# SamShue/EKF_SLAM

Measured on AMD Instinct MI355X. Metric: EKF update-steps/sec at N landmarks; HBM GB/s on (I−KH)P vs roofline, higher is better.
Workload: dtype f64

## Files before the change

### ekf_slam_amd/csrc/abi.hip

```cpp
#include "../../include/ekfslam.h"

#include <hip/hip_runtime.h>

#include <dlfcn.h>

#include <cstdio>
#include <cstdlib>
#include <algorithm>
#include <cmath>
#include <cstring>
#include <new>
#include <string>
#include <vector>

#include "device_math.h"
#include "flush32_pipe.h"
#include "kernels.h"
#include "layout.h"

struct KernelTimer {
    bool enabled = false;
    std::vector<hipEvent_t> ev;
    size_t used = 0;
};
// ... 38 lines not shown
    int32_t storage = 0;
    int32_t cur = 0;
    int32_t batch = 1;
    int32_t npend = 0;
    int32_t pstart = 0;
    bool async_flush = false;
    void *tilebuf[2] = { nullptr, nullptr };
    int32_t base = 0;
    int32_t nfrozen = 0;
    bool inflight = false;
    hipStream_t flush_stream = nullptr;
    hipEvent_t ev_pairs = nullptr, ev_flushed = nullptr, ev_rows = nullptr;
    hipEvent_t ev_xchg = nullptr;
    bool have_pp = false;
    PredictArgs pp;
    std::vector<double> s_host;
    mutable std::vector<std::pair<double, int64_t>> s_sorted, s_tail;
    mutable bool s_sorted_ok = false;
    static constexpr size_t kSortedTail = 2048;
    hipEvent_t throttle_ev[2] = { nullptr, nullptr };
    bool throttle_set[2] = { false, false };
    int throttle_k = 0, since_mark = 0;
    DevState st;
    hipStream_t own_stream = nullptr, stream = nullptr;
    int2 *d_work = nullptr;
    int64_t nwork = 0, work_rows = -1, work_cap = 0;
    char *wl_stage = nullptr;
    size_t wl_stage_bytes = 0;
    hipEvent_t ev_wl = nullptr;
    bool wl_busy = false;
// ... 234 lines not shown
    const bool alternate = force >= 0 ? force != 0 : store > kCacheBytes;
    h->st.tm.reverse = alternate ? (h->st.tm.reverse ^ 1) : 0;
}

int64_t slab_for(const ekf_handle *h, int64_t mm_rows) {
    const int64_t nt = ekf_tiles_for(mm_rows, h->T);
    const int64_t cmax = (nt + h->cfg.world - 1) / h->cfg.world;
    return cmax * h->T * 2;
}

double *corr_send(const ekf_handle *h, int64_t slab) {
    return (h->comm && h->send == h->own_send && h->recv == h->own_recv) ? h->recv + (size_t)h->cfg.rank * (size_t)slab : h->send;
}

int32_t exchange_rccl(ekf_handle *h);
int32_t flush_pending(ekf_handle *h, bool batch_done = false) {
    int32_t rc = retire_inflight(h);
    if (rc) return rc;
    if (h->npend == 0) return EKF_OK;
    rc = refresh_work(h);
    if (rc) return rc;
    next_pass_direction(h);
    bool extracted = false;
    const int64_t hint = h->hint_idx;
    bool pn = false, pn_side = false;
    if (batch_done && !h->pn_idx.empty()) {
        if (h->sharded && !h->pending && h->pn_N == h->N && (h->comm || h->xhook)) {
            const int32_t m = (int32_t)h->pn_idx.size();
            const int64_t slab = slab_for(h, n_mm(h));
            {
                TimedLaunch tl(h, EKF_KERNEL_ROWPANEL);
                HIPCHK(h, launch_rowpanel_next(h->st, h->pn_idx.data(), m, n_mm(h), h->pstart, h->npend, h->send, slab, h->storage, h->stream));
// ... 44 lines not shown
                                  h->storage, h->grid_cap, h->stream, h->dd_kernel, nx.j >= 0 ? &nx : nullptr, &extracted, h->cfg.pass_arith,
                                  h->d_segs ? &h->aux : nullptr));
        h->dd_pairs = h->npend;
    }
    h->npend = 0;
    h->pstart = 0;
    h->pf_valid = pn;
    if (pn_side) HIPCHK(h, hipStreamWaitEvent(h->stream, h->ev_pn_done, 0));
    h->nx_valid = extracted && !pn;
    if (extracted) { h->nx_idx = hint; h->nx_N = h->N; }
    return EKF_OK;
}

int32_t batch_complete(ekf_handle *h) {
    if (!h->async_flush) return flush_pending(h,  true);
    HIPCHK(h, hipEventRecord(h->ev_pairs, h->stream));
    int32_t rc = retire_inflight(h);
    if (rc) return rc;
    rc = refresh_work(h);
    if (rc) return rc;
    HIPCHK(h, hipStreamWaitEvent(h->flush_stream, h->ev_pairs, 0));
    {
        KernelTimer *t = &h->timers[EKF_KERNEL_DOWNDATE];
        hipEvent_t stop = nullptr;
        if (t->enabled) {
            if (t->used + 2 > t->ev.size()) {
                hipEvent_t a, b;
                HIPCHK(h, hipEventCreate(&a)); HIPCHK(h, hipEventCreate(&b));
                t->ev.push_back(a); t->ev.push_back(b);
            }
// ... 48 lines not shown
            continue;
        }
        const bool same = sp.is_new ? v.index == -1 : (int64_t)v.index == sp.idx;
        if (!same) {
            char buf[200];
            snprintf(buf, sizeof buf, "measure: the device association decided %s %d where the host mirror of the signatures "
                     "predicted %s %lld; the state is no longer the reference's", v.index == -1 ? "new landmark" : v.index == -2 ?
                     "(stale winner entries)" : "landmark", (int)v.index, sp.is_new ? "new landmark" : "landmark", (long long)sp.idx);
            rc = fail(h, EKF_ERR_STATE, buf);
        }
    }
    h->lspec.erase(h->lspec.begin(), h->lspec.begin() + (ptrdiff_t)done);
    return rc;
}

int32_t materialize_predict(ekf_handle *h) {
    if (!h->have_pp) return EKF_OK;
    h->have_pp = false;
    PredictArgs a = h->pp;
    a.n_mm = n_mm(h); a.cur = h->cur;
    {
        TimedLaunch tl(h, EKF_KERNEL_PREDICT);
        HIPCHK(h, launch_predict(h->st, a, h->storage, h->stream));
    }
    h->cur ^= 1;
    return EKF_OK;
}

int32_t do_predict(ekf_handle *h, const double u[2]) {
    int32_t rc = materialize_predict(h);
    if (rc) return rc;
// ... 1 lines not shown
    h->have_pp = true;
    static const bool lazy = ekf_tune_int("EKF_LAZY_PREDICT", 1) != 0;
    return lazy ? EKF_OK : materialize_predict(h);
}

int32_t enter(ekf_handle *h) {
    HIPCHK(h, hipSetDevice(h->cfg.device));
    const int32_t rc = verify_loop(h,  true);
    if (rc) return rc;
    return materialize_predict(h);
}

int32_t do_append(ekf_handle *h, const double u[2], const double R[4], const double pos[2], double signature,
                  const DevLoopArgs *dl = nullptr) {
    REQUIRE(h, h->N < h->cap, EKF_ERR_CAPACITY, "append: capacity_landmarks exhausted");
    if (h->inflight) h->appended_inflight = true;
    AppendArgs a;
    a.u0 = u[0]; a.u1 = u[1];
    colmajor2(R, a.R00, a.R01, a.R10, a.R11);
    a.pos0 = pos[0]; a.pos1 = pos[1]; a.signature = signature; a.N = h->N; a.cur = h->cur;
    {
        PredictArgs pa = h->pp;
        pa.n_mm = n_mm(h); pa.cur = h->cur;
        const PredictArgs *fuse = h->have_pp ? &pa : nullptr;
        TimedLaunch tl(h, EKF_KERNEL_APPEND);
        HIPCHK(h, launch_append(h->st, a, h->storage, h->stream, dl, fuse));
        if (fuse) { h->have_pp = false; h->cur ^= 1; }
    }
    if ((int64_t)h->s_host.size() > h->N) { h->s_host.resize((size_t)h->N); h->s_sorted_ok = false; }
    h->s_host.push_back(signature);
    if (h->s_sorted_ok && signature == signature)
        h->s_tail.emplace_back(signature, h->N);
    h->N += 1;
    h->pf_valid = false;
    h->nx_valid = false;
    h->pn_idx.clear();
// ... 134 lines not shown
        }
        int32_t rc = correct_begin(h, z, R, idx);
        if (rc) return rc;
        rc = exchange_rccl(h);
        if (rc) { h->pending = false; return rc; }
        return correct_finish(h);
    }
    REQUIRE(h, idx >= 0 && idx < h->N, EKF_ERR_INDEX, "correct: landmark index outside the state");
    int32_t rc = refresh_work(h);
    if (rc) return rc;
    CorrectArgs a;
    fill_correct_args(h, a, z, R, idx);
    static const bool fuse_small = ekf_tune_int("EKF_FUSE_SMALL", 1) != 0;
    const bool fused = fuse_small && h->batch == 1 && !h->async_flush && h->npend == 0 && a.n_mm <= gather_fuse_max_rows() &&
                       ekf_tiles_for(a.n_mm, h->T) * h->T <= 256;
    {
        TimedLaunch tl(h, EKF_KERNEL_GATHER);
        const PredictArgs *fuse = h->have_pp ? &h->pp : nullptr;
        HIPCHK(h, launch_gather(h->st, a, fuse, h->storage, h->stream, fused));
        h->have_pp = false;
    }
    if (fused) {
        h->cur ^= 1;
        h->st.dcur ^= 1;
        snprintf(h->dd_kernel, sizeof h->dd_kernel, "k_gather<%s,fused downdate>", h->storage == EKF_STORE_F64 ? "double" : "float");
        h->dd_pairs = 1;
        return throttle_step(h);
    }
    return finish_step(h);
}

int32_t do_correct_dev(ekf_handle *h, const double z[2], const double R[4], int64_t idx, const DevLoopArgs &dl) {
    REQUIRE(h, idx >= 0 && idx < h->N, EKF_ERR_INDEX, "correct: landmark index outside the state");
    int32_t rc = refresh_work(h);
    if (rc) return rc;
    CorrectArgs a;
    fill_correct_args(h, a, z, R, idx);
    if (h->sharded) {
        REQUIRE(h, !h->pending, EKF_ERR_STATE, "correct: an exchange is pending");
        h->slab = slab_for(h, a.n_mm);
        {
            TimedLaunch tl(h, EKF_KERNEL_ROWPANEL);
            HIPCHK(h, launch_rowpanel_dev(h->st, a.j, a.n_mm, h->pstart, h->npend, corr_send(h, h->slab), h->storage, h->stream, dl));
        }
        h->nx_valid = false;
        h->pending = true; h->pending_kind = 1; h->x_count = h->slab;
        rc = exchange_rccl(h);
        h->pending = false; h->pending_kind = 0;
        if (rc) return rc;
// ... 51 lines not shown
    return EKF_OK;
}

int32_t collect_decision(ekf_handle *h, AssocHostPartial *set, int32_t nblk, int32_t seq, int64_t N, bool may_poll, int32_t *is_new,
                         int64_t *idx) {
    if (!(may_poll && h->assoc_poll && wait_parts(set, nblk, seq))) {
        HIPCHK(h, hipStreamSynchronize(h->stream));
        __atomic_thread_fence(__ATOMIC_ACQUIRE);
    }
    return reduce_parts(h, set, nblk, seq, N, is_new, idx);
}

int32_t launch_assoc(ekf_handle *h, const double z[3], const double R[4], AssocHostPartial *host_set_dev, int32_t seq,
                     bool exchange = false, bool want_costs = false, bool fold_predict = false) {
    REQUIRE(h, h->N >= 1, EKF_ERR_STATE, "associate: the state holds no landmark (Correspondence.m:29)");
    if (!fold_predict) {
        const int32_t rcp = materialize_predict(h);
        if (rcp) return rcp;
    }
    AssocArgs a;
    a.z0 = z[0]; a.z1 = z[1]; a.z2 = z[2];
    colmajor2(R, a.R00, a.R01, a.R10, a.R11);
    a.s_cost = h->cfg.s_cost; a.s_thresh = h->cfg.s_thresh; a.w_pos = h->cfg.w_pos;
    a.N = h->N; a.cur = h->cur; a.npend = h->npend; a.pstart = h->pstart;
    a.own_only = exchange ? 1 : 0;
    TimedLaunch tl(h, EKF_KERNEL_ASSOCIATE);
    HIPCHK(h, launch_associate(h->st, a, exchange ? (want_costs ? h->send + 4 : nullptr) : h->d_pos_cost, h->d_sig_cost,
                               h->d_partial, h->d_ticket, h->d_decision, exchange ? nullptr : host_set_dev, seq,
                               exchange ? h->send : nullptr, h->storage, h->stream, (fold_predict && h->have_pp) ? &h->pp : nullptr));
    if (fold_predict && h->have_pp) { h->have_pp = false; h->cur ^= 1; }
// ... 1109 lines not shown
```

### ekf_slam_amd/csrc/append.h

```cpp
#pragma once

template <typename TS, bool kPredict = false>
__global__ __launch_bounds__(kBlock) void k_append(DevState st, AppendArgs a, DevLoopArgs dl, PredictArgs pa) {
    __shared__ PredictSmall aps;
    const int cur = a.cur;
    const int out = kPredict ? (cur ^ 1) : cur;
    if constexpr (kPredict) {
        if (threadIdx.x == 0) {
            const double pose[3] = { st.x[cur][0], st.x[cur][1], st.x[cur][2] };
            double prr_in[9];
            for (int i = 0; i < 9; ++i) prr_in[i] = st.prr[cur][i];
            predict_small(pose, prr_in, pa.u0, pa.u1, pa.C, aps);
        }
        __syncthreads();
    }
    if (dl.parts_in != nullptr && blockIdx.x == 0 && threadIdx.x < 64) {
        double dll;
        int dix;
        reduce_partials_wave(dl.parts_in, dl.nblk_in, dl.seq_in, (int)threadIdx.x, dll, dix);
        if (threadIdx.x == 0) store_partial(dl.rec, dll, dix, dl.seq_rec);
    }
    double *__restrict__ x = st.x[out];
    double *__restrict__ s = st.strip[out];
    const double *__restrict__ prr = kPredict ? aps.prr : st.prr[cur];
    TS *__restrict__ tiles = (TS *)st.tiles;
    const int64_t n_mm = 2 * a.N;
    const int64_t c = (int64_t)blockIdx.x * kBlock + threadIdx.x;
    const double th = kPredict ? aps.pose[2] : x[2];
    const double jxr[2][3] = { { 1, 0, -a.u0 * ekfm::sind(th) }, { 0, 1, a.u0 * ekfm::cosd(th) } };
    if (c < n_mm) {
        const double *__restrict__ sin_ = st.strip[cur];
        double s0 = sin_[c], s1 = sin_[st.ldm + c];
        const double s2 = sin_[2 * st.ldm + c];
        if constexpr (kPredict) {
            predict_strip(s0, s1, s2, aps.fa, aps.fb);
            s[c] = s0; s[st.ldm + c] = s1; s[2 * st.ldm + c] = s2;
            x[3 + c] = st.x[cur][3 + c];
        }
        for (int i = 0; i < 2; ++i) {
            const double v = jxr[i][0] * s0 + jxr[i][1] * s1 + jxr[i][2] * s2;
            if (st.tm.mine((n_mm + i) >> st.tm.shift, c >> st.tm.shift))
                pmm_low_store<TS>(tiles, st.tm, n_mm + i, c, v);
        }
    }
    if (c == 0) {
        if constexpr (kPredict) {
            for (int i = 0; i < 9; ++i) { st.prr[out][i] = aps.prr[i]; st.small[12 + i] = aps.Q[i]; }
            for (int i = 0; i < 3; ++i) x[i] = aps.pose[i];
        }
        x[3 + n_mm] = a.pos0;
        x[3 + n_mm + 1] = a.pos1;
        st.s[a.N] = a.signature;
        const double jz[2][2] = { { ekfm::cosd(a.u1), -a.u0 * ekfm::sind(a.u1) },
                                  { ekfm::sind(a.u1),  a.u0 * ekfm::cosd(a.u1) } };
        const double R[2][2] = { { a.R00, a.R01 }, { a.R10, a.R11 } };
        double t[2][3], c1[2][2], t2[2][2], c2[2][2];
        for (int i = 0; i < 2; ++i) for (int j = 0; j < 3; ++j) {
            double acc = 0; for (int k = 0; k < 3; ++k) acc += jxr[i][k] * prr[3 * k + j]; t[i][j] = acc; }
        for (int i = 0; i < 2; ++i) for (int j = 0; j < 2; ++j) {
            double acc = 0; for (int k = 0; k < 3; ++k) acc += t[i][k] * jxr[j][k]; c1[i][j] = acc; }
        for (int i = 0; i < 2; ++i) for (int j = 0; j < 2; ++j) {
            double acc = 0; for (int k = 0; k < 2; ++k) acc += jz[i][k] * R[k][j]; t2[i][j] = acc; }
        for (int i = 0; i < 2; ++i) for (int j = 0; j < 2; ++j) {
            double acc = 0; for (int k = 0; k < 2; ++k) acc += t2[i][k] * jz[j][k]; c2[i][j] = acc; }
        {
            double *__restrict__ dg = st.diag[st.dcur] + 3 * a.N;
            dg[0] = c1[0][0] + c2[0][0]; dg[1] = c1[1][0] + c2[1][0]; dg[2] = c1[1][1] + c2[1][1];
        }
        if (st.tm.mine(n_mm >> st.tm.shift, n_mm >> st.tm.shift)) {
            pmm_low_store<TS>(tiles, st.tm, n_mm, n_mm, c1[0][0] + c2[0][0]);
            pmm_low_store<TS>(tiles, st.tm, n_mm + 1, n_mm, c1[1][0] + c2[1][0]);
            pmm_low_store<TS>(tiles, st.tm, n_mm + 1, n_mm + 1, c1[1][1] + c2[1][1]);
        }
        for (int i = 0; i < 3; ++i) for (int j = 0; j < 2; ++j) {
            double acc = 0; for (int k = 0; k < 3; ++k) acc += prr[3 * i + k] * jxr[j][k];
            s[i * st.ldm + n_mm + j] = acc; }
    }
}
```

### ekf_slam_amd/csrc/gather.h

```cpp
#pragma once

constexpr int kGatherCols = 256;
constexpr int kGatherBlock = kGatherCols + 3 * 64;

__device__ __forceinline__ double lane_bcast(double v, int src) {
    const int lo = __builtin_amdgcn_readlane(__double2loint(v), src), hi = __builtin_amdgcn_readlane(__double2hiint(v), src);
    return __hiloint2double(hi, lo);
}
__device__ __forceinline__ double lane_gather(double v, int src) {
    const int lo = __builtin_amdgcn_ds_bpermute(src << 2, __double2loint(v)), hi = __builtin_amdgcn_ds_bpermute(src << 2, __double2hiint(v));
    return __hiloint2double(hi, lo);
}
__device__ __forceinline__ double lane_xor1(double v) {
    const int lo = __builtin_amdgcn_mov_dpp(__double2loint(v), 0xB1, 0xF, 0xF, true), hi = __builtin_amdgcn_mov_dpp(__double2hiint(v), 0xB1, 0xF, 0xF, true);
    return __hiloint2double(hi, lo);
}
__device__ __forceinline__ void wave_lds_sync() { asm volatile("s_waitcnt lgkmcnt(0)" ::: "memory"); }

constexpr int kFuseMaxRows = 48;
constexpr int kFuseElems = kFuseMaxRows * kFuseMaxRows / 256;

template <typename TS, bool kSharded, bool kPredict, bool kFused = false, bool kDev = false>
__global__ __launch_bounds__(kGatherBlock) void k_gather(DevState st, CorrectArgs a, PanelView pv, PredictArgs pa,
                                                         typename DevLoopParam<kDev>::type dl) {
    static_assert(!kDev || !kFused, "the device loop never drives the small-map fused form");
    __shared__ double pss[24];
    __shared__ SmallSolve sol;
    __shared__ PredictSmall ps;
    __shared__ double pose_sh[3];
    __shared__ int diag_ready;
    __shared__ int staged_cnt;
    __shared__ double2 upatch[kMaxPending * 4];
    const int tid = threadIdx.x;
    const int role = __builtin_amdgcn_readfirstlane(tid >> 6);
    const int lane = tid & 63;
    const int cur = a.cur;
    const double *__restrict__ x = cur ? st.x[1] : st.x[0];
    const double *__restrict__ strip = cur ? st.strip[1] : st.strip[0];
    const double *__restrict__ prr_cur = cur ? st.prr[1] : st.prr[0];
    double *__restrict__ x_nxt = cur ? st.x[0] : st.x[1];
    double *__restrict__ strip_nxt = cur ? st.strip[0] : st.strip[1];
    double *__restrict__ prr_nxt = cur ? st.prr[0] : st.prr[1];
    const TS *__restrict__ tiles = (const TS *)st.tiles;
    int64_t j = a.j;
    const int64_t ldm = st.ldm;
    const int npend = a.npend, pstart = a.pstart;
    if constexpr (kDev) {
        double dll;
        int dix;
        reduce_partials_wave(dl.parts_in, dl.nblk_in, dl.seq_in, lane, dll, dix);
        dix = __builtin_amdgcn_readfirstlane(dix);
        if (dix >= 0 && 2 * (int64_t)dix < a.n_mm) j = 2 * (int64_t)dix;
        if constexpr (kSharded) pv.Ij = j >> st.tm.shift;
        if (blockIdx.x == 0 && tid == kGatherCols + 128) store_partial(dl.rec, dll, dix, dl.seq_rec);
    }

    {
        const double *t_tiles = (const double *)st.tiles;
        asm volatile("" :: "s"(st.ldm), "s"(st.pair_stride), "s"(st.pcap), "s"(st.Gp), "s"(st.Kp), "s"(t_tiles), "s"(st.small),
                     "s"(st.tm.T), "s"(st.tm.shift), "s"(st.tm.world), "s"(st.tm.rank), "s"(a.j), "s"(a.n_mm), "s"(a.npend),
                     "s"(a.pstart));
// ... 4 lines not shown
#define EKF_STAMP() do { stamp[nst++] = clock64(); } while (0)
    EKF_STAMP();
#else
#define EKF_STAMP() do { } while (0)
#endif

    if (role >= 4) {
        double small_v = 0.0;
        if (role == 4) {
            const double *sp = prr_cur;
            if (lane < 9) sp = prr_cur + lane;
            else if (lane < 15) { const int t = (lane - 9) >> 1, b = (lane - 9) & 1; sp = strip + t * ldm + j + b; }
            else if (lane >= 19 && lane < 22) sp = x + (lane - 19);
            else if (lane >= 22 && lane < 24) sp = x + 3 + j + (lane - 22);
            small_v = *sp;
            if (lane == 24) { diag_ready = 0; staged_cnt = 0; }
        } else if (role == 5) {
            const int t = (lane >> 1) & 1, b = lane & 1;
            small_v = st.diag[st.dcur][3 * (j >> 1) + (t > b ? t : b) + (t > b ? b : t)];
        } else {
            small_v = x[lane < 3 ? lane : 3 + j + ((lane - 3) & 1)];
        }
        __builtin_amdgcn_sched_barrier(0);
        asm volatile("s_barrier" ::: "memory");
        EKF_STAMP();
        if (role == 4 && (lane < 15 || (lane >= 19 && lane < 24))) pss[lane] = small_v;
        if (role == 5 && lane < 4) pss[15 + lane] = small_v;
        EKF_STAMP();
        if (role == 5) {
            wave_lds_sync();
            if (lane == 0) *(volatile int *)&diag_ready = 1;
            EKF_STAMP();
        } else if (role == 6) {
            const double bx = lane_bcast(small_v, 0), by = lane_bcast(small_v, 1), bth = lane_bcast(small_v, 2),
                         blx = lane_bcast(small_v, 3), bly = lane_bcast(small_v, 4);
            if (lane == 0) {
                double pose[3] = { bx, by, bth };
                if (kPredict) {
                    const double2 sc2 = sincosd_ni(pose[2] + pa.u1);
                    const double sn2 = sc2.x, cs2 = sc2.y;
                    const double p0 = predict_pose_entry(pose, 0, pa.u0, pa.u1, sn2, cs2), p1 = predict_pose_entry(pose, 1, pa.u0, pa.u1, sn2, cs2),
                                 p2 = predict_pose_entry(pose, 2, pa.u0, pa.u1, sn2, cs2);
                    pose[0] = p0; pose[1] = p1; pose[2] = p2;
                }
                const double d0 = blx - pose[0], d1 = bly - pose[1];
                const double bearing = bearing_ni(d1, d0, pose[2]);
                const double sq = sqrt(d0 * d0 + d1 * d1);
                sol.nu[0] = a.z0 - sq;
                sol.nu[1] = a.z1 - bearing;
            }
        } else {
            double p[24];
#pragma unroll
            for (int i = 0; i < 24; ++i) p[i] = (i >= 15 && i < 19) ? 0.0 : lane_bcast(small_v, i);
// ... 17 lines not shown
                const double wj = EKF_SEL(ej == 0) ? W[0] : (EKF_SEL(ej == 1) ? W[1] : W[2]);
                double e_prr, e_q;
                predict_prr_entry(ei, ej, cj, c2, fa, fb, wi, wj, pa.C, e_prr, e_q);
                double s0 = v0, s1 = v1;
                predict_strip(s0, s1, v2, fa, fb);
                const double e_strip = EKF_SEL(st_t == 0) ? s0 : (EKF_SEL(st_t == 1) ? s1 : v2);
                const double p0 = predict_pose_entry(pose, 0, pa.u0, pa.u1, sn2, cs2), p1 = predict_pose_entry(pose, 1, pa.u0, pa.u1, sn2, cs2),
                             p2 = predict_pose_entry(pose, 2, pa.u0, pa.u1, sn2, cs2);
                pose[0] = p0; pose[1] = p1; pose[2] = p2;
                EKF_STAMP();
                if (lane < 15) pss[lane] = EKF_SEL(is_prr) ? e_prr : e_strip;
                if (lane < 9) ps.Q[lane] = e_q;
                if (lane == 0) { ps.fa = fa; ps.fb = fb; }
            }
            if (lane < 3) pose_sh[lane] = lane == 0 ? pose[0] : lane == 1 ? pose[1] : pose[2];
            SmallSolve so;
            double sq;
            solve_hs(p[22] - pose[0], p[23] - pose[1], sq, so.Hs);
            EKF_STAMP();
            while (*(volatile int *)&diag_ready == 0) { }
            wave_lds_sync();
            const int ra = lane >= 5 ? 1 : 0;
            double hsel[5];
#pragma unroll
            for (int t = 0; t < 5; ++t) hsel[t] = ra ? so.Hs[1][t] : so.Hs[0][t];
            const double e_gs = solve_gs_entry(pss, hsel, lane < 10 ? lane - 5 * ra : 0);
            double GS[2][5];
#pragma unroll
            for (int i = 0; i < 10; ++i) GS[i / 5][i % 5] = lane_bcast(e_gs, i);
            double e_phi;
            {
                const int aa = (lane >> 1) & 1, bb = lane & 1;
                double gsel[5], hb[5];
#pragma unroll
                for (int t = 0; t < 5; ++t) { gsel[t] = aa ? GS[1][t] : GS[0][t]; hb[t] = bb ? so.Hs[1][t] : so.Hs[0][t]; }
                const double Rab = aa == 0 ? (bb == 0 ? a.R00 : a.R01) : (bb == 0 ? a.R10 : a.R11);
// ... 67 lines not shown
        else if (rowpart) {
            const int64_t m = st.tm.T - 1;
            const TS *__restrict__ tp = tiles + st.tm.tile_offset(j >> st.tm.shift, c >> st.tm.shift) + ((j & m) << st.tm.shift) + (c & m);
            m0 = (double)tp[0]; m1 = (double)tp[st.tm.T];
        }
        else if (colpart) pmm_low_pair<TS>(tiles, st.tm, c, j, m0, m1);
        else pmm_low_pair<TS>(tiles, st.tm, j + 1, j, m0, m1);
        s0 = strip[c]; s1 = strip[ldm + c]; s2 = strip[2 * ldm + c];
        xc = x[3 + c];
    }
    double dgc = 0.0, dgl = 0.0;
    if (live) {
        const double *__restrict__ dg = st.diag[st.dcur] + 3 * (c >> 1);
        if (c & 1) { dgl = dg[1]; dgc = dg[2]; } else dgc = dg[0];
    }
    __builtin_amdgcn_sched_barrier(0);
    EKF_STAMP();
    upatch[tid] = up0; upatch[tid + kGatherCols] = up1;
    wave_lds_sync();
    if ((tid & 63) == 0) atomicAdd(&staged_cnt, 1);
    while (*(volatile int *)&staged_cnt < 4) { }
    wave_lds_sync();
    EKF_STAMP();

    constexpr int kPre = 32;
    const int npre = do_patch ? (npend < kPre ? npend : kPre) : 0;
    const int64_t pad_cols = st.tm.padded(a.n_mm);
    const int64_t ps2 = st.pair_stride / 2;
    double2 pre[kPre];
    bool next_assoc = false;
// ... 86 lines not shown
            for (int i = 0; i < npend; ++i) {
                m0 = rank2_apply(m0, upatch[4 * i + 1], upatch[4 * i + 2]);
                m1 = rank2_apply(m1, upatch[4 * i + 1], upatch[4 * i + 3]);
            }
        }
    }
    {
        const double dgl_p = lane_xor1(dgl);
        if (c == j) { m0 = dgc; m1 = dgl_p; }
        else if (c == j + 1) { m0 = dgl; m1 = dgc; }
    }
    EKF_STAMP();
    __syncthreads();
    EKF_STAMP();

    const int64_t pad_end = st.tm.padded(a.n_mm);
    const int64_t out_off = (int64_t)ring_slot(pstart, npend, st.pcap) * st.pair_stride;
    double2 *__restrict__ Gout = reinterpret_cast<double2 *>(st.Gp + out_off);
    double2 *__restrict__ Kout = reinterpret_cast<double2 *>(st.Kp + out_off);
    double g[2] = { 0.0, 0.0 }, k0 = 0.0, k1 = 0.0;
    double xn = 0.0, t0 = 0.0, t1 = 0.0, t2 = 0.0;
    if (live) {
        if (kPredict) predict_strip(s0, s1, s2, ps.fa, ps.fb);
        for (int r = 0; r < 2; ++r)
            g[r] = sol.Hs[r][0] * s0 + sol.Hs[r][1] * s1 + sol.Hs[r][2] * s2 + sol.Hs[r][3] * m0 + sol.Hs[r][4] * m1;
        k0 = g[0] * sol.Phi[0] + g[1] * sol.Phi[2];
        k1 = g[0] * sol.Phi[1] + g[1] * sol.Phi[3];
        if (!kFused) {
            Gout[c] = make_double2(g[0], g[1]);
            Kout[c] = make_double2(k0, k1);
            if (st.Gp32) {
                st.Gp32[out_off + c] = (float)g[0]; st.Gp32[out_off + ldm + c] = (float)g[1];
                st.Kp32[out_off + c] = -(float)k0; st.Kp32[out_off + ldm + c] = -(float)k1;
            }
        }
        xn = xc + (k0 * sol.nu[0] + k1 * sol.nu[1]);
        t0 = s0 - (sol.Kr[0][0] * g[0] + sol.Kr[0][1] * g[1]);
        t1 = s1 - (sol.Kr[1][0] * g[0] + sol.Kr[1][1] * g[1]);
// ... 107 lines not shown
```

### ekf_slam_amd/csrc/kernels.h

```cpp
#pragma once
#include <hip/hip_runtime.h>
#include <stdint.h>

#include <vector>

#include "layout.h"

#ifdef EKF_TUNING
#include <stdlib.h>
inline int ekf_tune_int(const char *name, int dflt) { const char *v = getenv(name); return v ? atoi(v) : dflt; }
#else
constexpr int ekf_tune_int(const char *, int dflt) { return dflt; }
#endif

struct DevState {
    double *x[2];
    double *prr[2];
    double *strip[2];
    void   *tiles;
    double *s;
    double *Gp;
    double *Kp;
    float  *Gp32;
    float  *Kp32;
// ... 67 lines not shown
    AssocHostPartial *rec;
    AssocHostPartial *parts_out;
    int32_t nblk_in, seq_in;
    int32_t seq_rec, seq_out;
    double z0, z1, z2;
    double R00, R01, R10, R11;
    double s_cost, s_thresh, w_pos;
};

constexpr int kAssocBlock = 256;

hipError_t launch_predict(const DevState &st, const PredictArgs &a, int storage, hipStream_t s);
hipError_t launch_append(const DevState &st, const AppendArgs &a, int storage, hipStream_t s, const DevLoopArgs *dl = nullptr,
                         const PredictArgs *fused_predict = nullptr);
hipError_t launch_gather(const DevState &st, const CorrectArgs &a, const PredictArgs *fused_predict, int storage,
                         hipStream_t s, bool fuse_downdate);
int gather_fuse_max_rows();
hipError_t launch_gather_devloop(const DevState &st, const CorrectArgs &a, const PredictArgs *fused_predict, const DevLoopArgs &dl,
                                 int storage, hipStream_t s);
int64_t gather_workgroups(const DevState &st, int64_t n_mm);
struct RowList { int32_t m; int32_t j[64]; };

hipError_t launch_rowpanel_base(const DevState &st, const int64_t *idx, int m, int64_t n_mm, double *send, int64_t slab,
                                int storage, hipStream_t s);
hipError_t launch_rowpanel_next(const DevState &st, const int64_t *idx, int m, int64_t n_mm, int pstart, int npend, double *send,
                                int64_t slab, int storage, hipStream_t s);
hipError_t launch_rowpanel(const DevState &st, int64_t j, int64_t n_mm, int pstart, int npend, double *send, int storage,
                           hipStream_t s);
hipError_t launch_rowpanel_dev(const DevState &st, int64_t j, int64_t n_mm, int pstart, int npend, double *send, int storage,
                               hipStream_t s, const DevLoopArgs &dl);
hipError_t launch_gather_sharded(const DevState &st, const CorrectArgs &a, const PredictArgs *fused_predict, const double *recv,
// ... 34 lines not shown
```

### ekf_slam_amd/csrc/kernels.hip

```cpp
#include "kernels.h"

#include <algorithm>
#include <atomic>
#include <cstdio>
#include <cstdlib>

#include "device_math.h"
#include "flush32_mfma.h"
#include "flush32_pipe.h"
#include "flush32_split.h"

namespace {

#include "tile_access.h"
#include "predict.h"
#include "assoc_winners.h"
#include "append.h"
#include "solve_small.h"
#include "rowpanel.h"
#include "gather.h"
#include "downdate.h"
#include "associate.h"
#include "state_io.h"

// ... 29 lines not shown
    PredictArgs pa = {};
    if (fused_predict) {
        pa = *fused_predict;
        EKF_STORAGE_DISPATCH(storage,
            hipLaunchKernelGGL((k_append<double, true>), dim3((unsigned)grid), dim3(kBlock), 0, s, st, a, dl, pa),
            hipLaunchKernelGGL((k_append<float, true>), dim3((unsigned)grid), dim3(kBlock), 0, s, st, a, dl, pa));
    } else {
        EKF_STORAGE_DISPATCH(storage,
            hipLaunchKernelGGL((k_append<double, false>), dim3((unsigned)grid), dim3(kBlock), 0, s, st, a, dl, pa),
            hipLaunchKernelGGL((k_append<float, false>), dim3((unsigned)grid), dim3(kBlock), 0, s, st, a, dl, pa));
    }
    return hipGetLastError();
}

hipError_t launch_gather(const DevState &st, const CorrectArgs &a, const PredictArgs *fused_predict, int storage,
                         hipStream_t s, bool fuse_downdate) {
    const int64_t cols = ekf_tiles_for(a.n_mm, st.tm.T) * st.tm.T;
    const int64_t grid = cdiv(cols, kGatherCols);
    PanelView pv;
    pv.recv = nullptr; pv.slab = 0; pv.offset = 0; pv.Ij = 0; pv.patched = 0;
    PredictArgs pa = {};
    if (fused_predict) pa = *fused_predict;
#define EKF_G(TS_, PRED_, FUSE_) hipLaunchKernelGGL((k_gather<TS_, false, PRED_, FUSE_>), dim3((unsigned)grid), dim3(kGatherBlock), 0, s, st, a, pv, pa, NoDevLoop{})
    if (fuse_downdate) {
        if (a.n_mm > kFuseMaxRows || grid != 1) return hipErrorInvalidValue;
        if (storage == 0) { if (fused_predict) EKF_G(double, true, true); else EKF_G(double, false, true); }
        else              { if (fused_predict) EKF_G(float, true, true); else EKF_G(float, false, true); }
    } else {
        if (storage == 0) { if (fused_predict) EKF_G(double, true, false); else EKF_G(double, false, false); }
        else              { if (fused_predict) EKF_G(float, true, false); else EKF_G(float, false, false); }
    }
#undef EKF_G
    return hipGetLastError();
}

int64_t gather_workgroups(const DevState &st, int64_t n_mm) { return cdiv(ekf_tiles_for(n_mm, st.tm.T) * st.tm.T, kGatherCols); }

hipError_t launch_gather_devloop(const DevState &st, const CorrectArgs &a, const PredictArgs *fused_predict, const DevLoopArgs &dl,
                                 int storage, hipStream_t s) {
    if (!dl.parts_in || !dl.rec || dl.nblk_in < 1 || a.n_mm < 2) return hipErrorInvalidValue;
    const int64_t grid = gather_workgroups(st, a.n_mm);
    PanelView pv;
    pv.recv = nullptr; pv.slab = 0; pv.offset = 0; pv.Ij = 0; pv.patched = 0;
    PredictArgs pa = {};
    if (fused_predict) pa = *fused_predict;
#define EKF_G(TS_, PRED_) hipLaunchKernelGGL((k_gather<TS_, false, PRED_, false, true>), dim3((unsigned)grid), dim3(kGatherBlock), 0, s, st, a, pv, pa, dl)
    if (storage == 0) { if (fused_predict) EKF_G(double, true); else EKF_G(double, false); }
    else              { if (fused_predict) EKF_G(float, true); else EKF_G(float, false); }
#undef EKF_G
    return hipGetLastError();
}

hipError_t launch_rowpanel(const DevState &st, int64_t j, int64_t n_mm, int pstart, int npend, double *send, int storage,
                           hipStream_t s) {
    const int64_t nloc = rowpanel_local_chunks(st.tm, j, n_mm);
    if (nloc == 0) return hipSuccess;
    const int64_t grid = cdiv(nloc * st.tm.T, kBlock);
    EKF_STORAGE_DISPATCH(storage,
        hipLaunchKernelGGL(k_rowpanel<double>, dim3((unsigned)grid), dim3(kBlock), 0, s, st, j, n_mm, pstart, npend, send, nloc, NoDevLoop{}),
        hipLaunchKernelGGL(k_rowpanel<float>, dim3((unsigned)grid), dim3(kBlock), 0, s, st, j, n_mm, pstart, npend, send, nloc, NoDevLoop{}));
    return hipGetLastError();
// ... 43 lines not shown
        hipLaunchKernelGGL(k_rowpanel_base<double>, dim3((unsigned)grid, (unsigned)m), dim3(kBlock), 0, s, st, rows, n_mm, send, slab),
        hipLaunchKernelGGL(k_rowpanel_base<float>, dim3((unsigned)grid, (unsigned)m), dim3(kBlock), 0, s, st, rows, n_mm, send, slab));
    return hipGetLastError();
}

hipError_t launch_gather_sharded(const DevState &st, const CorrectArgs &a, const PredictArgs *fused_predict, const double *recv,
                                 int64_t rank_stride, int64_t offset, bool patched, int storage, hipStream_t s, const DevLoopArgs *dl) {
    const int64_t cols = ekf_tiles_for(a.n_mm, st.tm.T) * st.tm.T;
    const int64_t grid = cdiv(cols, kGatherCols);
    PanelView pv;
    pv.recv = recv; pv.slab = rank_stride; pv.offset = offset; pv.Ij = a.j >> st.tm.shift; pv.patched = patched ? 1 : 0;
    PredictArgs pa = {};
    if (fused_predict) pa = *fused_predict;
    if (dl) {
        if (!dl->parts_in || !dl->rec || dl->nblk_in < 1 || a.n_mm < 2) return hipErrorInvalidValue;
#define EKF_GD(TS_, PRED_) hipLaunchKernelGGL((k_gather<TS_, true, PRED_, false, true>), dim3((unsigned)grid), dim3(kGatherBlock), 0, s, st, a, pv, pa, *dl)
        if (storage == 0) { if (fused_predict) EKF_GD(double, true); else EKF_GD(double, false); }
        else              { if (fused_predict) EKF_GD(float, true); else EKF_GD(float, false); }
#undef EKF_GD
        return hipGetLastError();
    }
#define EKF_G(TS_, PRED_) hipLaunchKernelGGL((k_gather<TS_, true, PRED_>), dim3((unsigned)grid), dim3(kGatherBlock), 0, s, st, a, pv, pa, NoDevLoop{})
    if (storage == 0) { if (fused_predict) EKF_G(double, true); else EKF_G(double, false); }
    else              { if (fused_predict) EKF_G(float, true); else EKF_G(float, false); }
#undef EKF_G
    return hipGetLastError();
}

#include "flush64_mfma.h"

static void name_kernel(char *out, const char *base, size_t elt, int T, int p3, int xcd) {
    if (!out) return;
    if (xcd < 0) snprintf(out, 64, "%s<%s,%d,%d>", base, elt == 8 ? "double" : "float", T, p3);
    else snprintf(out, 64, "%s<%s,%d,%d,%s>", base, elt == 8 ? "double" : "float", T, p3, xcd ? "true" : "false");
}

static hipError_t allow_dynamic_lds(const void *fn, size_t bytes, std::atomic<uint64_t> &done) {
// ... 344 lines not shown
```

Measured before the change: 1942.

## Defer landmark append and fold it into the following gather kernel

New-landmark appends are recorded on the host and launched lazily. When the next step is an unsharded, unfused gather, the append's covariance cross-terms, diagonal block and signature write are computed inside k_gather instead of a separate k_append launch. This removes one kernel launch and one pass over the pose strip per append. In exchange the gather kernel gains an extra template variant with more LDS, spin-wait handshakes and patched-value logic. All other entry points materialize any pending append first.

```diff
diff --git a/ekf_slam_amd/csrc/abi.hip b/ekf_slam_amd/csrc/abi.hip
--- a/ekf_slam_amd/csrc/abi.hip
+++ b/ekf_slam_amd/csrc/abi.hip
@@ -76,6 +76,10 @@
     hipEvent_t ev_xchg = nullptr;
     bool have_pp = false;
     PredictArgs pp;
+    bool have_app = false;
+    AppendArgs app;
+    bool app_pp = false;
+    PredictArgs app_pa;
     std::vector<double> s_host;
     mutable std::vector<std::pair<double, int64_t>> s_sorted, s_tail;
     mutable bool s_sorted_ok = false;
@@ -340,8 +344,11 @@
 }
 
 int32_t exchange_rccl(ekf_handle *h);
+int32_t materialize_append(ekf_handle *h);
 int32_t flush_pending(ekf_handle *h, bool batch_done = false) {
-    int32_t rc = retire_inflight(h);
+    int32_t rc = materialize_append(h);
+    if (rc) return rc;
+    rc = retire_inflight(h);
     if (rc) return rc;
     if (h->npend == 0) return EKF_OK;
     rc = refresh_work(h);
@@ -416,6 +423,10 @@
 
 int32_t batch_complete(ekf_handle *h) {
     if (!h->async_flush) return flush_pending(h,  true);
+    {
+        const int32_t rca = materialize_append(h);
+        if (rca) return rca;
+    }
     HIPCHK(h, hipEventRecord(h->ev_pairs, h->stream));
     int32_t rc = retire_inflight(h);
     if (rc) return rc;
@@ -494,7 +505,26 @@
     return rc;
 }
 
+int32_t materialize_append(ekf_handle *h) {
+    if (!h->have_app) return EKF_OK;
+    h->have_app = false;
+    AppendArgs a = h->app;
+    a.cur = h->cur;
+    PredictArgs pa = h->app_pa;
+    pa.cur = h->cur;
+    const PredictArgs *fuse = h->app_pp ? &pa : nullptr;
+    h->app_pp = false;
+    {
+        TimedLaunch tl(h, EKF_KERNEL_APPEND);
+        HIPCHK(h, launch_append(h->st, a, h->storage, h->stream, nullptr, fuse));
+    }
+    if (fuse) h->cur ^= 1;
+    return EKF_OK;
+}
+
 int32_t materialize_predict(ekf_handle *h) {
+    const int32_t rca = materialize_append(h);
+    if (rca) return rca;
     if (!h->have_pp) return EKF_OK;
     h->have_pp = false;
     PredictArgs a = h->pp;
@@ -526,12 +556,22 @@
 int32_t do_append(ekf_handle *h, const double u[2], const double R[4], const double pos[2], double signature,
                   const DevLoopArgs *dl = nullptr) {
     REQUIRE(h, h->N < h->cap, EKF_ERR_CAPACITY, "append: capacity_landmarks exhausted");
+    int32_t rc = materialize_append(h);
+    if (rc) return rc;
     if (h->inflight) h->appended_inflight = true;
     AppendArgs a;
     a.u0 = u[0]; a.u1 = u[1];
     colmajor2(R, a.R00, a.R01, a.R10, a.R11);
     a.pos0 = pos[0]; a.pos1 = pos[1]; a.signature = signature; a.N = h->N; a.cur = h->cur;
-    {
+    static const bool fold = ekf_tune_int("EKF_FOLD_APPEND", 1) != 0;
+    if (fold && !h->sharded && dl == nullptr) {
+        h->app = a;
+        h->app_pp = h->have_pp;
+        h->app_pa = h->pp;
+        h->app_pa.n_mm = n_mm(h); h->app_pa.cur = h->cur;
+        h->have_pp = false;
+        h->have_app = true;
+    } else {
         PredictArgs pa = h->pp;
         pa.n_mm = n_mm(h); pa.cur = h->cur;
         const PredictArgs *fuse = h->have_pp ? &pa : nullptr;
@@ -696,11 +736,19 @@
     static const bool fuse_small = ekf_tune_int("EKF_FUSE_SMALL", 1) != 0;
     const bool fused = fuse_small && h->batch == 1 && !h->async_flush && h->npend == 0 && a.n_mm <= gather_fuse_max_rows() &&
                        ekf_tiles_for(a.n_mm, h->T) * h->T <= 256;
+    if (fused) {
+        rc = materialize_append(h);
+        if (rc) return rc;
+        a.cur = h->cur;
+    }
     {
         TimedLaunch tl(h, EKF_KERNEL_GATHER);
-        const PredictArgs *fuse = h->have_pp ? &h->pp : nullptr;
-        HIPCHK(h, launch_gather(h->st, a, fuse, h->storage, h->stream, fused));
+        const bool with_app = h->have_app;
+        PredictArgs pa = h->app_pa;
+        const PredictArgs *fuse = with_app ? (h->app_pp ? &pa : nullptr) : (h->have_pp ? &h->pp : nullptr);
+        HIPCHK(h, launch_gather(h->st, a, fuse, h->storage, h->stream, fused, with_app ? &h->app : nullptr));
         h->have_pp = false;
+        h->have_app = false; h->app_pp = false;
     }
     if (fused) {
         h->cur ^= 1;
@@ -714,7 +762,9 @@
 
 int32_t do_correct_dev(ekf_handle *h, const double z[2], const double R[4], int64_t idx, const DevLoopArgs &dl) {
     REQUIRE(h, idx >= 0 && idx < h->N, EKF_ERR_INDEX, "correct: landmark index outside the state");
-    int32_t rc = refresh_work(h);
+    int32_t rc = materialize_append(h);
+    if (rc) return rc;
+    rc = refresh_work(h);
     if (rc) return rc;
     CorrectArgs a;
     fill_correct_args(h, a, z, R, idx);
@@ -796,6 +846,10 @@
 int32_t launch_assoc(ekf_handle *h, const double z[3], const double R[4], AssocHostPartial *host_set_dev, int32_t seq,
                      bool exchange = false, bool want_costs = false, bool fold_predict = false) {
     REQUIRE(h, h->N >= 1, EKF_ERR_STATE, "associate: the state holds no landmark (Correspondence.m:29)");
+    {
+        const int32_t rca = materialize_append(h);
+        if (rca) return rca;
+    }
     if (!fold_predict) {
         const int32_t rcp = materialize_predict(h);
         if (rcp) return rcp;
diff --git a/ekf_slam_amd/csrc/append.h b/ekf_slam_amd/csrc/append.h
--- a/ekf_slam_amd/csrc/append.h
+++ b/ekf_slam_amd/csrc/append.h
@@ -1,4 +1,38 @@
 #pragma once
+
+__device__ __forceinline__ void append_jxr(double u0, double sn, double cs, double jxr[2][3]) {
+    jxr[0][0] = 1; jxr[0][1] = 0; jxr[0][2] = -u0 * sn;
+    jxr[1][0] = 0; jxr[1][1] = 1; jxr[1][2] = u0 * cs;
+}
+__device__ __forceinline__ double append_row(const double ji[3], double s0, double s1, double s2) {
+    return ji[0] * s0 + ji[1] * s1 + ji[2] * s2;
+}
+__device__ __forceinline__ void append_c2(double u0, double snu, double csu, double R00, double R01, double R10, double R11,
+                                          double c2[2][2]) {
+    const double jz[2][2] = { { csu, -u0 * snu }, { snu, u0 * csu } };
+    const double R[2][2] = { { R00, R01 }, { R10, R11 } };
+    double t2[2][2];
+    for (int i = 0; i < 2; ++i) for (int j = 0; j < 2; ++j) {
+        double acc = 0; for (int k = 0; k < 2; ++k) acc += jz[i][k] * R[k][j]; t2[i][j] = acc; }
+    for (int i = 0; i < 2; ++i) for (int j = 0; j < 2; ++j) {
+        double acc = 0; for (int k = 0; k < 2; ++k) acc += t2[i][k] * jz[j][k]; c2[i][j] = acc; }
+}
+__device__ __forceinline__ void append_block(const double prr[9], const double jxr[2][3], const double c2[2][2], double dg[3],
+                                             double I[3][2]) {
+    double t[2][3], c1[2][2];
+    for (int i = 0; i < 2; ++i) for (int j = 0; j < 3; ++j) {
+        double acc = 0; for (int k = 0; k < 3; ++k) acc += jxr[i][k] * prr[3 * k + j]; t[i][j] = acc; }
+    for (int i = 0; i < 2; ++i) for (int j = 0; j < 2; ++j) {
+        double acc = 0; for (int k = 0; k < 3; ++k) acc += t[i][k] * jxr[j][k]; c1[i][j] = acc; }
+    dg[0] = c1[0][0] + c2[0][0]; dg[1] = c1[1][0] + c2[1][0]; dg[2] = c1[1][1] + c2[1][1];
+    for (int i = 0; i < 3; ++i) for (int j = 0; j < 2; ++j) {
+        double acc = 0; for (int k = 0; k < 3; ++k) acc += prr[3 * i + k] * jxr[j][k];
+        I[i][j] = acc; }
+}
+
+struct NoAppend {};
+template <bool kAppend> struct AppendParam { using type = NoAppend; };
+template <> struct AppendParam<true> { using type = AppendArgs; };
 
 template <typename TS, bool kPredict = false>
 __global__ __launch_bounds__(kBlock) void k_append(DevState st, AppendArgs a, DevLoopArgs dl, PredictArgs pa) {
@@ -27,7 +61,8 @@
     const int64_t n_mm = 2 * a.N;
     const int64_t c = (int64_t)blockIdx.x * kBlock + threadIdx.x;
     const double th = kPredict ? aps.pose[2] : x[2];
-    const double jxr[2][3] = { { 1, 0, -a.u0 * ekfm::sind(th) }, { 0, 1, a.u0 * ekfm::cosd(th) } };
+    double jxr[2][3];
+    append_jxr(a.u0, ekfm::sind(th), ekfm::cosd(th), jxr);
     if (c < n_mm) {
         const double *__restrict__ sin_ = st.strip[cur];
         double s0 = sin_[c], s1 = sin_[st.ldm + c];
@@ -38,7 +73,7 @@
             x[3 + c] = st.x[cur][3 + c];
         }
         for (int i = 0; i < 2; ++i) {
-            const double v = jxr[i][0] * s0 + jxr[i][1] * s1 + jxr[i][2] * s2;
+            const double v = append_row(jxr[i], s0, s1, s2);
             if (st.tm.mine((n_mm + i) >> st.tm.shift, c >> st.tm.shift))
                 pmm_low_store<TS>(tiles, st.tm, n_mm + i, c, v);
         }
@@ -51,29 +86,18 @@
         x[3 + n_mm] = a.pos0;
         x[3 + n_mm + 1] = a.pos1;
         st.s[a.N] = a.signature;
-        const double jz[2][2] = { { ekfm::cosd(a.u1), -a.u0 * ekfm::sind(a.u1) },
-                                  { ekfm::sind(a.u1),  a.u0 * ekfm::cosd(a.u1) } };
-        const double R[2][2] = { { a.R00, a.R01 }, { a.R10, a.R11 } };
-        double t[2][3], c1[2][2], t2[2][2], c2[2][2];
-        for (int i = 0; i < 2; ++i) for (int j = 0; j < 3; ++j) {
-            double acc = 0; for (int k = 0; k < 3; ++k) acc += jxr[i][k] * prr[3 * k + j]; t[i][j] = acc; }
-        for (int i = 0; i < 2; ++i) for (int j = 0; j < 2; ++j) {
-            double acc = 0; for (int k = 0; k < 3; ++k) acc += t[i][k] * jxr[j][k]; c1[i][j] = acc; }
-        for (int i = 0; i < 2; ++i) for (int j = 0; j < 2; ++j) {
-            double acc = 0; for (int k = 0; k < 2; ++k) acc += jz[i][k] * R[k][j]; t2[i][j] = acc; }
-        for (int i = 0; i < 2; ++i) for (int j = 0; j < 2; ++j) {
-            double acc = 0; for (int k = 0; k < 2; ++k) acc += t2[i][k] * jz[j][k]; c2[i][j] = acc; }
+        double c2[2][2], dg[3], I[3][2];
+        append_c2(a.u0, ekfm::sind(a.u1), ekfm::cosd(a.u1), a.R00, a.R01, a.R10, a.R11, c2);
+        append_block(prr, jxr, c2, dg, I);
         {
-            double *__restrict__ dg = st.diag[st.dcur] + 3 * a.N;
-            dg[0] = c1[0][0] + c2[0][0]; dg[1] = c1[1][0] + c2[1][0]; dg[2] = c1[1][1] + c2[1][1];
+            double *__restrict__ dgp = st.diag[st.dcur] + 3 * a.N;
+            dgp[0] = dg[0]; dgp[1] = dg[1]; dgp[2] = dg[2];
         }
         if (st.tm.mine(n_mm >> st.tm.shift, n_mm >> st.tm.shift)) {
-            pmm_low_store<TS>(tiles, st.tm, n_mm, n_mm, c1[0][0] + c2[0][0]);
-            pmm_low_store<TS>(tiles, st.tm, n_mm + 1, n_mm, c1[1][0] + c2[1][0]);
-            pmm_low_store<TS>(tiles, st.tm, n_mm + 1, n_mm + 1, c1[1][1] + c2[1][1]);
+            pmm_low_store<TS>(tiles, st.tm, n_mm, n_mm, dg[0]);
+            pmm_low_store<TS>(tiles, st.tm, n_mm + 1, n_mm, dg[1]);
+            pmm_low_store<TS>(tiles, st.tm, n_mm + 1, n_mm + 1, dg[2]);
         }
-        for (int i = 0; i < 3; ++i) for (int j = 0; j < 2; ++j) {
-            double acc = 0; for (int k = 0; k < 3; ++k) acc += prr[3 * i + k] * jxr[j][k];
-            s[i * st.ldm + n_mm + j] = acc; }
+        for (int i = 0; i < 3; ++i) for (int j = 0; j < 2; ++j) s[i * st.ldm + n_mm + j] = I[i][j];
     }
 }
diff --git a/ekf_slam_amd/csrc/gather.h b/ekf_slam_amd/csrc/gather.h
--- a/ekf_slam_amd/csrc/gather.h
+++ b/ekf_slam_amd/csrc/gather.h
@@ -17,13 +17,18 @@
 }
 __device__ __forceinline__ void wave_lds_sync() { asm volatile("s_waitcnt lgkmcnt(0)" ::: "memory"); }
 
+__device__ __forceinline__ double append_patched(double v, double zneg) {
+    return ((v == 0.0 && signbit(v)) || zneg != zneg) ? zneg : v;
+}
+
 constexpr int kFuseMaxRows = 48;
 constexpr int kFuseElems = kFuseMaxRows * kFuseMaxRows / 256;
 
-template <typename TS, bool kSharded, bool kPredict, bool kFused = false, bool kDev = false>
+template <typename TS, bool kSharded, bool kPredict, bool kFused = false, bool kDev = false, bool kAppend = false>
 __global__ __launch_bounds__(kGatherBlock) void k_gather(DevState st, CorrectArgs a, PanelView pv, PredictArgs pa,
-                                                         typename DevLoopParam<kDev>::type dl) {
+                                                         typename DevLoopParam<kDev>::type dl, typename AppendParam<kAppend>::type ap) {
     static_assert(!kDev || !kFused, "the device loop never drives the small-map fused form");
+    static_assert(!kAppend || (!kSharded && !kFused && !kDev), "the append is folded into the unsharded, unfused gather only");
     __shared__ double pss[24];
     __shared__ SmallSolve sol;
     __shared__ PredictSmall ps;
@@ -31,6 +36,8 @@
     __shared__ int diag_ready;
     __shared__ int staged_cnt;
     __shared__ double2 upatch[kMaxPending * 4];
+    __shared__ double app_small[6];
+    __shared__ int app_ready;
     const int tid = threadIdx.x;
     const int role = __builtin_amdgcn_readfirstlane(tid >> 6);
     const int lane = tid & 63;
@@ -45,6 +52,9 @@
     int64_t j = a.j;
     const int64_t ldm = st.ldm;
     const int npend = a.npend, pstart = a.pstart;
+    int64_t nA = 0;
+    if constexpr (kAppend) nA = 2 * ap.N;
+    const bool newlm = kAppend && j == nA;
     if constexpr (kDev) {
         double dll;
         int dix;
@@ -79,7 +89,7 @@
             else if (lane >= 19 && lane < 22) sp = x + (lane - 19);
             else if (lane >= 22 && lane < 24) sp = x + 3 + j + (lane - 22);
             small_v = *sp;
-            if (lane == 24) { diag_ready = 0; staged_cnt = 0; }
+            if (lane == 24) { diag_ready = 0; staged_cnt = 0; if constexpr (kAppend) app_ready = 0; }
         } else if (role == 5) {
             const int t = (lane >> 1) & 1, b = lane & 1;
             small_v = st.diag[st.dcur][3 * (j >> 1) + (t > b ? t : b) + (t > b ? b : t)];
@@ -97,12 +107,30 @@
             if (lane == 0) *(volatile int *)&diag_ready = 1;
             EKF_STAMP();
         } else if (role == 6) {
-            const double bx = lane_bcast(small_v, 0), by = lane_bcast(small_v, 1), bth = lane_bcast(small_v, 2),
-                         blx = lane_bcast(small_v, 3), bly = lane_bcast(small_v, 4);
+            const double bx = lane_bcast(small_v, 0), by = lane_bcast(small_v, 1), bth = lane_bcast(small_v, 2);
+            double blx = lane_bcast(small_v, 3), bly = lane_bcast(small_v, 4);
+            double2 sc_app = make_double2(0.0, 0.0);
+            if constexpr (kAppend) {
+                const double pose0[3] = { bx, by, bth };
+                const double thp = kPredict ? predict_pose_entry(pose0, 2, pa.u0, pa.u1, 0.0, 0.0) : bth;
+                sc_app = sincosd_ni(lane == 0 ? bth + pa.u1 : lane == 1 ? thp : ap.u1);
+                const double snt = lane_bcast(sc_app.x, 1), cst = lane_bcast(sc_app.y, 1), snu = lane_bcast(sc_app.x, 2),
+                             csu = lane_bcast(sc_app.y, 2);
+                if (lane == 0) {
+                    double jxr[2][3], c2[2][2];
+                    append_jxr(ap.u0, snt, cst, jxr);
+                    append_c2(ap.u0, snu, csu, ap.R00, ap.R01, ap.R10, ap.R11, c2);
+                    app_small[0] = jxr[0][2]; app_small[1] = jxr[1][2];
+                    app_small[2] = c2[0][0]; app_small[3] = c2[0][1]; app_small[4] = c2[1][0]; app_small[5] = c2[1][1];
+                    wave_lds_sync();
+                    *(volatile int *)&app_ready = 1;
+                }
+                if (newlm) { blx = ap.pos0; bly = ap.pos1; }
+            }
             if (lane == 0) {
                 double pose[3] = { bx, by, bth };
                 if (kPredict) {
-                    const double2 sc2 = sincosd_ni(pose[2] + pa.u1);
+                    const double2 sc2 = kAppend ? sc_app : sincosd_ni(pose[2] + pa.u1);
                     const double sn2 = sc2.x, cs2 = sc2.y;
                     const double p0 = predict_pose_entry(pose, 0, pa.u0, pa.u1, sn2, cs2), p1 = predict_pose_entry(pose, 1, pa.u0, pa.u1, sn2, cs2),
                                  p2 = predict_pose_entry(pose, 2, pa.u0, pa.u1, sn2, cs2);
@@ -150,12 +178,33 @@
                 if (lane == 0) { ps.fa = fa; ps.fb = fb; }
             }
             if (lane < 3) pose_sh[lane] = lane == 0 ? pose[0] : lane == 1 ? pose[1] : pose[2];
+            if constexpr (kAppend) if (newlm) { p[22] = ap.pos0; p[23] = ap.pos1; }
             SmallSolve so;
             double sq;
             solve_hs(p[22] - pose[0], p[23] - pose[1], sq, so.Hs);
             EKF_STAMP();
             while (*(volatile int *)&diag_ready == 0) { }
             wave_lds_sync();
+            if constexpr (kAppend) {
+                if (newlm) {
+                    while (*(volatile int *)&app_ready == 0) { }
+                    wave_lds_sync();
+                    double prr[9], jxr[2][3], c2[2][2], dg[3], I[3][2];
+#pragma unroll
+                    for (int i = 0; i < 9; ++i) prr[i] = pss[i];
+                    jxr[0][0] = 1; jxr[0][1] = 0; jxr[0][2] = app_small[0];
+                    jxr[1][0] = 0; jxr[1][1] = 1; jxr[1][2] = app_small[1];
+                    c2[0][0] = app_small[2]; c2[0][1] = app_small[3]; c2[1][0] = app_small[4]; c2[1][1] = app_small[5];
+                    append_block(prr, jxr, c2, dg, I);
+                    wave_lds_sync();
+                    if (lane == 0) {
+#pragma unroll
+                        for (int t = 0; t < 3; ++t) { pss[9 + 2 * t] = I[t][0]; pss[10 + 2 * t] = I[t][1]; }
+                        pss[15] = dg[0]; pss[16] = dg[1]; pss[17] = dg[1]; pss[18] = dg[2];
+                    }
+                    wave_lds_sync();
+                }
+            }
             const int ra = lane >= 5 ? 1 : 0;
             double hsel[5];
 #pragma unroll
@@ -253,6 +302,8 @@
         const double *__restrict__ dg = st.diag[st.dcur] + 3 * (c >> 1);
         if (c & 1) { dgl = dg[1]; dgc = dg[2]; } else dgc = dg[0];
     }
+    const bool app_entry = kAppend && live && (c >= nA || newlm);
+    if (app_entry) { m0 = -0.0; m1 = -0.0; }
     __builtin_amdgcn_sched_barrier(0);
     EKF_STAMP();
     upatch[tid] = up0; upatch[tid + kGatherCols] = up1;
@@ -369,6 +420,48 @@
     __syncthreads();
     EKF_STAMP();
 
+    if constexpr (kAppend) {
+        const bool newcol = c >= nA;
+        double jxr[2][3];
+        jxr[0][0] = 1; jxr[0][1] = 0; jxr[0][2] = app_small[0];
+        jxr[1][0] = 0; jxr[1][1] = 1; jxr[1][2] = app_small[1];
+        TS *__restrict__ tw = (TS *)st.tiles;
+        if (live && !newcol) {
+            if (kPredict) predict_strip(s0, s1, s2, ps.fa, ps.fb);
+            const double r0 = append_row(jxr[0], s0, s1, s2), r1 = append_row(jxr[1], s0, s1, s2);
+            const int64_t m = st.tm.T - 1;
+            TS *__restrict__ tp = tw + st.tm.tile_offset(nA >> st.tm.shift, c >> st.tm.shift) + ((nA & m) << st.tm.shift) + (c & m);
+            tp[0] = (TS)r0;
+            tp[st.tm.T] = (TS)r1;
+            if (newlm) { m0 = append_patched((double)(TS)r0, m0); m1 = append_patched((double)(TS)r1, m1); }
+        } else if (live) {
+            const int b = (int)(c - nA);
+            double prr[9], c2[2][2], dg[3], I[3][2];
+#pragma unroll
+            for (int i = 0; i < 9; ++i) prr[i] = pss[i];
+            c2[0][0] = app_small[2]; c2[0][1] = app_small[3]; c2[1][0] = app_small[4]; c2[1][1] = app_small[5];
+            append_block(prr, jxr, c2, dg, I);
+            s0 = b ? I[0][1] : I[0][0]; s1 = b ? I[1][1] : I[1][0]; s2 = b ? I[2][1] : I[2][0];
+            xc = b ? ap.pos1 : ap.pos0;
+            dgc = b ? dg[2] : dg[0]; dgl = b ? dg[1] : 0.0;
+            if (b == 0) {
+                pmm_low_store<TS>(tw, st.tm, nA, nA, dg[0]);
+                st.s[ap.N] = ap.signature;
+            } else {
+                pmm_low_store<TS>(tw, st.tm, nA + 1, nA, dg[1]);
+                pmm_low_store<TS>(tw, st.tm, nA + 1, nA + 1, dg[2]);
+            }
+            if (!newlm) {
+                const double *ji = b ? jxr[1] : jxr[0];
+                m0 = append_patched((double)(TS)append_row(ji, pss[9], pss[11], pss[13]), m0);
+                m1 = append_patched((double)(TS)append_row(ji, pss[10], pss[12], pss[14]), m1);
+            }
+        }
+        const double dgl_p = lane_xor1(dgl);
+        if (newlm && c == j) { m0 = dgc; m1 = dgl_p; }
+        else if (newlm && c == j + 1) { m0 = dgl; m1 = dgc; }
+    }
+
     const int64_t pad_end = st.tm.padded(a.n_mm);
     const int64_t out_off = (int64_t)ring_slot(pstart, npend, st.pcap) * st.pair_stride;
     double2 *__restrict__ Gout = reinterpret_cast<double2 *>(st.Gp + out_off);
@@ -376,7 +469,7 @@
     double g[2] = { 0.0, 0.0 }, k0 = 0.0, k1 = 0.0;
     double xn = 0.0, t0 = 0.0, t1 = 0.0, t2 = 0.0;
     if (live) {
-        if (kPredict) predict_strip(s0, s1, s2, ps.fa, ps.fb);
+        if (kPredict && !kAppend) predict_strip(s0, s1, s2, ps.fa, ps.fb);
         for (int r = 0; r < 2; ++r)
             g[r] = sol.Hs[r][0] * s0 + sol.Hs[r][1] * s1 + sol.Hs[r][2] * s2 + sol.Hs[r][3] * m0 + sol.Hs[r][4] * m1;
         k0 = g[0] * sol.Phi[0] + g[1] * sol.Phi[2];
diff --git a/ekf_slam_amd/csrc/kernels.h b/ekf_slam_amd/csrc/kernels.h
--- a/ekf_slam_amd/csrc/kernels.h
+++ b/ekf_slam_amd/csrc/kernels.h
@@ -105,7 +105,7 @@
 hipError_t launch_append(const DevState &st, const AppendArgs &a, int storage, hipStream_t s, const DevLoopArgs *dl = nullptr,
                          const PredictArgs *fused_predict = nullptr);
 hipError_t launch_gather(const DevState &st, const CorrectArgs &a, const PredictArgs *fused_predict, int storage,
-                         hipStream_t s, bool fuse_downdate);
+                         hipStream_t s, bool fuse_downdate, const AppendArgs *fused_append = nullptr);
 int gather_fuse_max_rows();
 hipError_t launch_gather_devloop(const DevState &st, const CorrectArgs &a, const PredictArgs *fused_predict, const DevLoopArgs &dl,
                                  int storage, hipStream_t s);
diff --git a/ekf_slam_amd/csrc/kernels.hip b/ekf_slam_amd/csrc/kernels.hip
--- a/ekf_slam_amd/csrc/kernels.hip
+++ b/ekf_slam_amd/csrc/kernels.hip
@@ -67,14 +67,23 @@
 }
 
 hipError_t launch_gather(const DevState &st, const CorrectArgs &a, const PredictArgs *fused_predict, int storage,
-                         hipStream_t s, bool fuse_downdate) {
+                         hipStream_t s, bool fuse_downdate, const AppendArgs *fused_append) {
     const int64_t cols = ekf_tiles_for(a.n_mm, st.tm.T) * st.tm.T;
     const int64_t grid = cdiv(cols, kGatherCols);
     PanelView pv;
     pv.recv = nullptr; pv.slab = 0; pv.offset = 0; pv.Ij = 0; pv.patched = 0;
     PredictArgs pa = {};
     if (fused_predict) pa = *fused_predict;
-#define EKF_G(TS_, PRED_, FUSE_) hipLaunchKernelGGL((k_gather<TS_, false, PRED_, FUSE_>), dim3((unsigned)grid), dim3(kGatherBlock), 0, s, st, a, pv, pa, NoDevLoop{})
+    if (fused_append) {
+        const AppendArgs &ap = *fused_append;
+        if (fuse_downdate || st.tm.world != 1 || a.n_mm != 2 * (ap.N + 1) || a.j < 0 || a.j > 2 * ap.N) return hipErrorInvalidValue;
+#define EKF_GA(TS_, PRED_) hipLaunchKernelGGL((k_gather<TS_, false, PRED_, false, false, true>), dim3((unsigned)grid), dim3(kGatherBlock), 0, s, st, a, pv, pa, NoDevLoop{}, ap)
+        if (storage == 0) { if (fused_predict) EKF_GA(double, true); else EKF_GA(double, false); }
+        else              { if (fused_predict) EKF_GA(float, true); else EKF_GA(float, false); }
+#undef EKF_GA
+        return hipGetLastError();
+    }
+#define EKF_G(TS_, PRED_, FUSE_) hipLaunchKernelGGL((k_gather<TS_, false, PRED_, FUSE_>), dim3((unsigned)grid), dim3(kGatherBlock), 0, s, st, a, pv, pa, NoDevLoop{}, NoAppend{})
     if (fuse_downdate) {
         if (a.n_mm > kFuseMaxRows || grid != 1) return hipErrorInvalidValue;
         if (storage == 0) { if (fused_predict) EKF_G(double, true, true); else EKF_G(double, false, true); }
@@ -97,7 +106,7 @@
     pv.recv = nullptr; pv.slab = 0; pv.offset = 0; pv.Ij = 0; pv.patched = 0;
     PredictArgs pa = {};
     if (fused_predict) pa = *fused_predict;
-#define EKF_G(TS_, PRED_) hipLaunchKernelGGL((k_gather<TS_, false, PRED_, false, true>), dim3((unsigned)grid), dim3(kGatherBlock), 0, s, st, a, pv, pa, dl)
+#define EKF_G(TS_, PRED_) hipLaunchKernelGGL((k_gather<TS_, false, PRED_, false, true>), dim3((unsigned)grid), dim3(kGatherBlock), 0, s, st, a, pv, pa, dl, NoAppend{})
     if (storage == 0) { if (fused_predict) EKF_G(double, true); else EKF_G(double, false); }
     else              { if (fused_predict) EKF_G(float, true); else EKF_G(float, false); }
 #undef EKF_G
@@ -171,13 +180,13 @@
     if (fused_predict) pa = *fused_predict;
     if (dl) {
         if (!dl->parts_in || !dl->rec || dl->nblk_in < 1 || a.n_mm < 2) return hipErrorInvalidValue;
-#define EKF_GD(TS_, PRED_) hipLaunchKernelGGL((k_gather<TS_, true, PRED_, false, true>), dim3((unsigned)grid), dim3(kGatherBlock), 0, s, st, a, pv, pa, *dl)
+#define EKF_GD(TS_, PRED_) hipLaunchKernelGGL((k_gather<TS_, true, PRED_, false, true>), dim3((unsigned)grid), dim3(kGatherBlock), 0, s, st, a, pv, pa, *dl, NoAppend{})
         if (storage == 0) { if (fused_predict) EKF_GD(double, true); else EKF_GD(double, false); }
         else              { if (fused_predict) EKF_GD(float, true); else EKF_GD(float, false); }
 #undef EKF_GD
         return hipGetLastError();
     }
-#define EKF_G(TS_, PRED_) hipLaunchKernelGGL((k_gather<TS_, true, PRED_>), dim3((unsigned)grid), dim3(kGatherBlock), 0, s, st, a, pv, pa, NoDevLoop{})
+#define EKF_G(TS_, PRED_) hipLaunchKernelGGL((k_gather<TS_, true, PRED_>), dim3((unsigned)grid), dim3(kGatherBlock), 0, s, st, a, pv, pa, NoDevLoop{}, NoAppend{})
     if (storage == 0) { if (fused_predict) EKF_G(double, true); else EKF_G(double, false); }
     else              { if (fused_predict) EKF_G(float, true); else EKF_G(float, false); }
 #undef EKF_G
```

After: 1939 (median of 5 runs). Within noise of the previous version (-0.2%).
